# dherrera1911/sqfa

Hardware: AMD Instinct MI355X
Metric: SPD pairwise-distance loss+grad evals/sec (higher is better)
Workload: dtype f32; 1 GPU; c3: C=1000 classes, n_dim=784, n_filters=16, smsqfa (m=16), 499500 unordered pairs per eval, inputs resident in HBM; parallelism=pair-tile shard over 1 GPU(s) + 1 all-reduce of [loss,flags,grad] per eval

## Files before the change

sqfa_amd/csrc/pair_inst.hip:

```cpp
#include <type_traits>

#include "configs.hpp"
#include "pair_kernel.hpp"

#define SQFA_CAT_(a, b, c) a##b##_##c
#define SQFA_CAT(a, b, c) SQFA_CAT_(a, b, c)

#if defined(SQFA_RS) && SQFA_RS != 0
#include "pair_kernel_2d.hpp"
#define SQFA_ROW2D_MATCHES(T, MR, GC, CPL, TJ, WV, RS) \
  || (std::is_same<T, SQFA_T>::value && MR == SQFA_MR && GC == SQFA_G && CPL == SQFA_CPL && TJ == SQFA_TJ && WV == SQFA_WAVES && RS == SQFA_RS)
static_assert(false SQFA_CONFIGS2D_F32(SQFA_ROW2D_MATCHES) SQFA_CONFIGS2D_F64(SQFA_ROW2D_MATCHES),
              "Makefile CONFIGS2D and configs.hpp disagree");
namespace sqfa {
hipError_t SQFA_CAT(launch_pair2d_, SQFA_TAG, SQFA_MR)(const PairParams& p, hipStream_t stream) {
  return launch_pair_tiles_2d<PairCfg2D<SQFA_T, SQFA_MR, SQFA_G, SQFA_CPL, SQFA_TJ, SQFA_WAVES, SQFA_RS>>(p, stream);
}
hipError_t SQFA_CAT(launch_pair2d_bw_, SQFA_TAG, SQFA_MR)(const PairParams& p, hipStream_t stream) {
  return launch_pair_tiles_2d_bw<PairCfg2D<SQFA_T, SQFA_MR, SQFA_G, SQFA_CPL, SQFA_TJ, SQFA_WAVES, SQFA_RS>>(p, stream);
}
hipError_t SQFA_CAT(launch_factor2d_, SQFA_TAG, SQFA_MR)(const PairParams& p, hipStream_t stream) {
  return launch_class_factors<PairCfg2D<SQFA_T, SQFA_MR, SQFA_G, SQFA_CPL, SQFA_TJ, SQFA_WAVES, SQFA_RS>>(p, stream);
}
hipError_t SQFA_CAT(launch_classeig2d_, SQFA_TAG, SQFA_MR)(const void* LT, int n, int m, double* U, double* lam, hipStream_t stream) {
  return launch_class_eig<PairCfg2D<SQFA_T, SQFA_MR, SQFA_G, SQFA_CPL, SQFA_TJ, SQFA_WAVES, SQFA_RS>>(LT, n, m, U, lam, stream);
}
}
#else
#define SQFA_ROW_MATCHES(T, MR, G, CPL, TJ, WV) \
  || (std::is_same<T, SQFA_T>::value && MR == SQFA_MR && G == SQFA_G && CPL == SQFA_CPL && TJ == SQFA_TJ && WV == SQFA_WAVES)
static_assert(false SQFA_CONFIGS_F32(SQFA_ROW_MATCHES) SQFA_CONFIGS_F64(SQFA_ROW_MATCHES) SQFA_CONFIGS_F32_SMALL(SQFA_ROW_MATCHES)
              SQFA_CONFIGS_F64_SMALL(SQFA_ROW_MATCHES),
              "Makefile CONFIGS / CONFIGS_SMALL and configs.hpp disagree");
namespace sqfa {
hipError_t SQFA_CAT(launch_pair_, SQFA_TAG, SQFA_MR)(const PairParams& p, hipStream_t stream) {
  return launch_pair_tiles<PairCfg<SQFA_T, SQFA_MR, SQFA_G, SQFA_CPL, SQFA_TJ, SQFA_WAVES>>(p, stream);
}
hipError_t SQFA_CAT(launch_pair_bw_, SQFA_TAG, SQFA_MR)(const PairParams& p, hipStream_t stream) {
  return launch_pair_tiles_bw<PairCfg<SQFA_T, SQFA_MR, SQFA_G, SQFA_CPL, SQFA_TJ, SQFA_WAVES>>(p, stream);
}
hipError_t SQFA_CAT(launch_factor_, SQFA_TAG, SQFA_MR)(const PairParams& p, hipStream_t stream) {
  return launch_class_factors<PairCfg<SQFA_T, SQFA_MR, SQFA_G, SQFA_CPL, SQFA_TJ, SQFA_WAVES>>(p, stream);
}
hipError_t SQFA_CAT(launch_classeig_, SQFA_TAG, SQFA_MR)(const void* LT, int n, int m, double* U, double* lam, hipStream_t stream) {
  return launch_class_eig<PairCfg<SQFA_T, SQFA_MR, SQFA_G, SQFA_CPL, SQFA_TJ, SQFA_WAVES>>(LT, n, m, U, lam, stream);
}
}
#endif
```

sqfa_amd/csrc/pair_kernel.hpp:

```cpp
#pragma once
#include <hip/hip_runtime.h>
#include <stdint.h>

namespace sqfa {

struct PairParams {
  const void* LT;
  const void* Linv;
  const void* W;
  const void* EW;
  void* slab_grad;
  void* slab_loss;
  int* slab_flag;
  int* row_start;
  void* dist_out;
  void* eig_out;
  unsigned long long* sweep_counter;
  int nA, nB, m;
  int self_mode, sqrt_mode, want_grad;
  int shard_index, shard_count;
  int nbi, nbj;
  int tj;
  int factor_mode;
  const double* mean_linv;
// ... 7 lines not shown
template <typename T> __device__ __forceinline__ T param_scale(const PairParams& p) {
  if constexpr (sizeof(T) == 4) return p.scale_f; else return p.scale;
}
template <typename T> __device__ __forceinline__ T param_eps(const PairParams& p) {
  if constexpr (sizeof(T) == 4) return p.eps_f; else return p.eps;
}
template <typename T> __device__ __forceinline__ T param_uniform_weight(const PairParams& p) {
  if constexpr (sizeof(T) == 4) return p.uniform_weight_f; else return p.uniform_weight;
}

__host__ __device__ inline int tiles_in_row(int bi, int nbj, int TI, int TJ, int self_mode) {
  if (!self_mode) return nbj;
  const int q = bi * TI + TI - 2;
  if (q < 0) return 0;
  const int len = q / TJ + 1;
  return len < nbj ? len : nbj;
}
__host__ __device__ inline int shard_tiles_in_row(int bi, int len, int shard_index, int shard_count, int* first) {
  const int o = ((shard_index - bi) % shard_count + shard_count) % shard_count;
  *first = o;
  return len > o ? (len - 1 - o) / shard_count + 1 : 0;
}

__device__ inline void write_row_start_table(const PairParams& pp, int TI, int* row_start) {
  __shared__ int s_cnt[256];
  int base = 0;
  for (int b0 = 0; b0 < pp.nbi; b0 += 256) {
    const int bi = b0 + (int)threadIdx.x;
    int cnt = 0, first;
    if (bi < pp.nbi)
      cnt = shard_tiles_in_row(bi, tiles_in_row(bi, pp.nbj, TI, pp.tj, pp.self_mode), pp.shard_index, pp.shard_count, &first);
    s_cnt[threadIdx.x] = cnt;
    __syncthreads();
    if (threadIdx.x == 0) {
      int acc = base;
      for (int k = 0; k < 256 && b0 + k < pp.nbi; ++k) {
        row_start[b0 + k] = acc;
        acc += s_cnt[k];
      }
      s_cnt[0] = acc;
    }
    __syncthreads();
    base = s_cnt[0];
    __syncthreads();
  }
  if (threadIdx.x == 0) row_start[pp.nbi] = base;
}

__host__ __device__ constexpr int ilog2(int v);
__host__ __device__ constexpr int pow2ceil(int v) {
  int p = 1;
  while (p < v) p <<= 1;
  return p;
}
__host__ __device__ constexpr int tri_index(int r, int c) { return r * (r + 1) / 2 + c; }

template <typename T> struct Real;
template <> struct Real<float> {
  static constexpr float kEps = 1.1920929e-07f;
// ... 1276 lines not shown
  return hipGetLastError();
}

template <typename Cfg>
hipError_t launch_pair_tiles(const PairParams& p, hipStream_t stream) {
  long n_tiles = 0;
  for (int bi = 0; bi < p.nbi; ++bi) {
    int first;
    n_tiles += shard_tiles_in_row(bi, tiles_in_row(bi, p.nbj, Cfg::TI, p.tj, p.self_mode), p.shard_index,
                                  p.shard_count, &first);
  }
  if (n_tiles == 0) return hipSuccess;
  dim3 grid((unsigned)n_tiles, 1, 1);
  using T = typename Cfg::type;
  if (p.EW != nullptr)
    hipLaunchKernelGGL((pair_tile_kernel<Cfg, true>), grid, dim3(Cfg::THREADS), 0, stream, p, static_cast<const T*>(p.LT),
                       static_cast<const T*>(p.Linv), static_cast<const T*>(p.W), static_cast<const T*>(p.EW));
  else
    hipLaunchKernelGGL((pair_tile_kernel<Cfg, false>), grid, dim3(Cfg::THREADS), 0, stream, p, static_cast<const T*>(p.LT),
                       static_cast<const T*>(p.Linv), static_cast<const T*>(p.W), static_cast<const T*>(p.EW));
  return hipGetLastError();
}

#ifndef SQFA_FACTOR_F64
#define SQFA_FACTOR_F64 1
#endif
template <typename Tio_, int MR_>
struct FactorCfg {
  using io_type = Tio_;
  static constexpr int MR = MR_;
#ifndef SQFA_FACTOR_G
  static constexpr int G = MR_ <= 24 ? 16 : 32;
#else
  static constexpr int G = SQFA_FACTOR_G;
#endif
  static constexpr int CPL = (MR_ + G - 1) / G;
  static constexpr int PPW = 64 / G;
};

template <typename T, int MR, int G, int CPL, int ROWS = MR>
__device__ __forceinline__ int class_jacobi_sweeps(T (&x)[CPL][ROWS], T (&D)[CPL], int max_sweeps) {
  using R = Real<T>;
  constexpr bool LONE = (MR == G * (CPL - 1) + 1);
  const T tol2 = R::kEps * R::kEps * T(MR);
  T nrm[CPL];
  int sweeps = 0;
  bool more = true;
  while (more && sweeps < max_sweeps) {
    {
// ... 38 lines not shown
            x[c2][r] = R::fma_(a2, xp, x[c2][r]);
          }
          D[c1] *= u;
          D[c2] *= u;
          nrm[c1] -= kg2;
          nrm[c2] += kg2;
        }
      }
    }
    constexpr int STATIC_G = sizeof(T) == 4 ? 32 : 16;
    if constexpr (G > 1 && G <= STATIC_G) {
      cross_rounds_static<T, ROWS, G, CPL, 1, LONE ? 1 : 0>(x, nrm, D, tol2, big);
    } else if constexpr (G > STATIC_G) {
#pragma unroll 1
      for (int s = 1; s < G; ++s) cross_round<T, ROWS, CPL, 0, 0, LONE>(x, nrm, D, s, tol2, big);
    }
    if constexpr (z_visits_cfg<G, MR, CPL>()) z_visits<T, ROWS, G, CPL, swizzled_rows_of_8<T, G, MR>(), 0>(x, nrm, D, tol2, big);
    more = __any(big);
    ++sweeps;
  }
  return sweeps;
}

template <typename Cfg>
__global__ __launch_bounds__(64) void class_factor_kernel(typename Cfg::io_type* __restrict__ LT, int nA, int max_sweeps) {
  using Tio = typename Cfg::io_type;
#if SQFA_FACTOR_F64
  using T = double;
#else
  using T = Tio;
#endif
  using R = Real<T>;
  constexpr int MR = Cfg::MR, G = Cfg::G, CPL = Cfg::CPL, PPW = Cfg::PPW;
  const int lane = threadIdx.x & 63;
  const int g = lane % G;
  const int cls = blockIdx.x * PPW + lane / G;
  Tio* lt = LT + (size_t)(cls < nA ? cls : nA - 1) * (MR * MR);
  T x[CPL][MR];
#pragma unroll
  for (int c = 0; c < CPL; ++c) {
    const int col = c * G + g;
    const Tio* src = lt + (size_t)(col < MR ? col : 0) * MR;
    const bool real_col = col < MR;
#pragma unroll
    for (int k = 0; k < MR; ++k) x[c][k] = real_col ? (T)src[k] : T(0);
  }
  T D[CPL];
#pragma unroll
  for (int c = 0; c < CPL; ++c) D[c] = T(1);
  class_jacobi_sweeps<T, MR, G, CPL>(x, D, max_sweeps);
  if (cls < nA) {
#pragma unroll
    for (int c = 0; c < CPL; ++c) {
      const int col = c * G + g;
      if (col < MR) {
        const T dc = R::sqrt_(D[c]);
        Tio* dst = lt + (size_t)col * MR;
#pragma unroll
        for (int r = 0; r < MR; ++r) dst[r] = (Tio)(x[c][r] * dc);
      }
    }
  }
}

template <typename Cfg>
__global__ __launch_bounds__(64) void class_factor_mean_kernel(typename Cfg::io_type* __restrict__ LT, int nA, int max_sweeps,
                                                               const double* __restrict__ mean_linv) {
  using Tio = typename Cfg::io_type;
  using T = double;
  using R = Real<T>;
  constexpr int MR = Cfg::MR, G = Cfg::G, CPL = Cfg::CPL, PPW = Cfg::PPW, ROWS = 2 * MR;
  constexpr T kStack = T(1.0 / (1 << 30)), kUnstack = T(1 << 30);
  __shared__ T s_li[MR * MR];
  const int lane = threadIdx.x & 63;
  for (int k = lane; k < MR * MR; k += 64) s_li[k] = mean_linv[k];
  __syncthreads();
  const int g = lane % G;
  const int cls = blockIdx.x * PPW + lane / G;
  Tio* lt = LT + (size_t)(cls < nA ? cls : nA - 1) * (MR * MR);
  T x[CPL][ROWS];
#pragma unroll
  for (int c = 0; c < CPL; ++c) {
// ... 64 lines not shown
        for (int r = 0; r < MR; ++r) a = R::fma_(x[c][r], x[c][r], a);
        const T l = a * D[c];
        lam[(size_t)cls * m + col] = l;
        const T inv = R::sqrt_(D[c]) / R::sqrt_(l);
#pragma unroll
        for (int r = 0; r < MR; ++r) {
          if (r < m) U[((size_t)cls * m + r) * m + col] = x[c][r] * inv;
        }
      }
    }
  }
}

template <typename Cfg>
hipError_t launch_class_eig(const void* LT, int n, int m, double* U, double* lam, hipStream_t stream) {
  using T = typename Cfg::type;
  using FC = FactorCfg<T, Cfg::MR>;
  const int blocks = (n + FC::PPW - 1) / FC::PPW;
  hipLaunchKernelGGL((class_eig_kernel<FC>), dim3(blocks), dim3(64), 0, stream, static_cast<const T*>(LT), n, m, U, lam);
  return hipGetLastError();
}

template <typename Cfg>
hipError_t launch_class_factors(const PairParams& p, hipStream_t stream) {
  if constexpr (!Cfg::DENSE_FACTOR) {
    return hipSuccess;
  } else {
    using T = typename Cfg::type;
    using FC = FactorCfg<T, Cfg::MR>;
    const long pairs = p.self_mode ? (long)p.nA * (p.nA - 1) / 2 : (long)p.nA * p.nB;
    if (p.factor_mode < 0 || (p.factor_mode == 0 && pairs / p.shard_count < Cfg::FACTOR_MIN_PAIRS)) return hipSuccess;
    const int blocks = (p.nA + FC::PPW - 1) / FC::PPW;
    if constexpr (Cfg::MEAN_METRIC) {
      if (p.mean_linv != nullptr) {
        hipLaunchKernelGGL((class_factor_mean_kernel<FC>), dim3(blocks), dim3(64), 0, stream,
                           static_cast<T*>(const_cast<void*>(p.LT)), p.nA, Cfg::FACTOR_SWEEPS, p.mean_linv);
        return hipGetLastError();
      }
    }
    hipLaunchKernelGGL((class_factor_kernel<FC>), dim3(blocks), dim3(64), 0, stream,
                       static_cast<T*>(const_cast<void*>(p.LT)), p.nA, Cfg::FACTOR_SWEEPS);
    return hipGetLastError();
  }
}

}
```

sqfa_amd/csrc/sqfa_api.hip:

```cpp
#include <hip/hip_runtime.h>
#include <stdio.h>
#include <string.h>

#include <algorithm>
#include <atomic>
#include <mutex>
#include <utility>
#include <vector>

#include "../../include/sqfa_hip.h"
#include "configs.hpp"
#include "pair_kernel.hpp"
#include "pair_kernel_2d.hpp"
#include "pair_kernel_lds.hpp"

namespace sqfa {

#define SQFA_DECL_F32(T, MR, G, CPL, TJ, WV) \
  hipError_t launch_pair_f32_##MR(const PairParams&, hipStream_t);   \
  hipError_t launch_pair_bw_f32_##MR(const PairParams&, hipStream_t); \
  hipError_t launch_factor_f32_##MR(const PairParams&, hipStream_t); \
  hipError_t launch_classeig_f32_##MR(const void*, int, int, double*, double*, hipStream_t);
#define SQFA_DECL_F64(T, MR, G, CPL, TJ, WV) \
  hipError_t launch_pair_f64_##MR(const PairParams&, hipStream_t);   \
  hipError_t launch_pair_bw_f64_##MR(const PairParams&, hipStream_t); \
  hipError_t launch_factor_f64_##MR(const PairParams&, hipStream_t); \
  hipError_t launch_classeig_f64_##MR(const void*, int, int, double*, double*, hipStream_t);
SQFA_CONFIGS_F32(SQFA_DECL_F32)
SQFA_CONFIGS_F64(SQFA_DECL_F64)
#define SQFA_DECL_F32S(T, MR, G, CPL, TJ, WV) \
  hipError_t launch_pair_f32s_##MR(const PairParams&, hipStream_t);  \
  hipError_t launch_pair_bw_f32s_##MR(const PairParams&, hipStream_t); \
  hipError_t launch_factor_f32s_##MR(const PairParams&, hipStream_t);
SQFA_CONFIGS_F32_SMALL(SQFA_DECL_F32S)
#define SQFA_DECL_F64S(T, MR, G, CPL, TJ, WV) \
  hipError_t launch_pair_f64s_##MR(const PairParams&, hipStream_t);  \
  hipError_t launch_pair_bw_f64s_##MR(const PairParams&, hipStream_t); \
  hipError_t launch_factor_f64s_##MR(const PairParams&, hipStream_t);
SQFA_CONFIGS_F64_SMALL(SQFA_DECL_F64S)

#define SQFA_DECL2D_F32(T, MR, GC, CPL, TJ, WV, RS) \
  hipError_t launch_pair2d_f32_##MR(const PairParams&, hipStream_t); \
  hipError_t launch_pair2d_bw_f32_##MR(const PairParams&, hipStream_t); \
  hipError_t launch_factor2d_f32_##MR(const PairParams&, hipStream_t); \
  hipError_t launch_classeig2d_f32_##MR(const void*, int, int, double*, double*, hipStream_t);
#define SQFA_DECL2D_F64(T, MR, GC, CPL, TJ, WV, RS) \
  hipError_t launch_pair2d_f64_##MR(const PairParams&, hipStream_t); \
  hipError_t launch_pair2d_bw_f64_##MR(const PairParams&, hipStream_t); \
  hipError_t launch_factor2d_f64_##MR(const PairParams&, hipStream_t); \
  hipError_t launch_classeig2d_f64_##MR(const void*, int, int, double*, double*, hipStream_t);
SQFA_CONFIGS2D_F32(SQFA_DECL2D_F32)
SQFA_CONFIGS2D_F64(SQFA_DECL2D_F64)

struct Geometry {
  int dtype, MR, TJ, TI, WV;
  hipError_t (*launch)(const PairParams&, hipStream_t);
  hipError_t (*factor)(const PairParams&, hipStream_t);
  hipError_t (*eig)(const void*, int, int, double*, double*, hipStream_t);
  hipError_t (*launch_bw)(const PairParams&, hipStream_t);
  bool mean_metric;
  long factor_min_pairs;
};
template <typename Cfg>
static Geometry make_geometry(decltype(Geometry::launch) launch, decltype(Geometry::factor) factor, decltype(Geometry::eig) eig,
                              decltype(Geometry::launch_bw) launch_bw) {
  return Geometry{sizeof(typename Cfg::type) == 4 ? SQFA_F32 : SQFA_F64, Cfg::MR, Cfg::TJ, Cfg::TI, Cfg::WAVES, launch, factor, eig,
                  launch_bw, Cfg::MEAN_METRIC, Cfg::FACTOR_MIN_PAIRS};
}

static bool find_geometry(int m, int dtype, long pairs, Geometry* out, int geometry_mode = 0) {
  bool found = false;
  Geometry best{};
  auto consider = [&](const Geometry& g) {
    if (g.dtype == dtype && m <= g.MR && (!found || g.MR < best.MR)) {
      best = g;
      found = true;
    }
  };
  auto consider_small = [&](Geometry g, long max_pairs) {
    g.eig = best.eig;
    if (g.dtype == dtype && g.MR == best.MR && (geometry_mode > 0 || pairs < max_pairs)) best = g;
  };
#define SQFA_ROW_F32(T, MR, G, CPL, TJ, WV) \
  consider(make_geometry<PairCfg<T, MR, G, CPL, TJ, WV>>(launch_pair_f32_##MR, launch_factor_f32_##MR, launch_classeig_f32_##MR, launch_pair_bw_f32_##MR));
#define SQFA_ROW_F64(T, MR, G, CPL, TJ, WV) \
  consider(make_geometry<PairCfg<T, MR, G, CPL, TJ, WV>>(launch_pair_f64_##MR, launch_factor_f64_##MR, launch_classeig_f64_##MR, launch_pair_bw_f64_##MR));
#define SQFA_ROW2D_F32(T, MR, GC, CPL, TJ, WV, RS) \
  consider(make_geometry<PairCfg2D<T, MR, GC, CPL, TJ, WV, RS>>(launch_pair2d_f32_##MR, launch_factor2d_f32_##MR, launch_classeig2d_f32_##MR, launch_pair2d_bw_f32_##MR));
#define SQFA_ROW2D_F64(T, MR, GC, CPL, TJ, WV, RS) \
  consider(make_geometry<PairCfg2D<T, MR, GC, CPL, TJ, WV, RS>>(launch_pair2d_f64_##MR, launch_factor2d_f64_##MR, launch_classeig2d_f64_##MR, launch_pair2d_bw_f64_##MR));
#define SQFA_ROW_F32S(T, MR, G, CPL, TJ, WV) \
  consider_small(make_geometry<PairCfg<T, MR, G, CPL, TJ, WV>>(launch_pair_f32s_##MR, launch_factor_f32s_##MR, nullptr, launch_pair_bw_f32s_##MR), small_launch_max_pairs(MR));
#define SQFA_ROW_F64S(T, MR, G, CPL, TJ, WV) \
  consider_small(make_geometry<PairCfg<T, MR, G, CPL, TJ, WV>>(launch_pair_f64s_##MR, launch_factor_f64s_##MR, nullptr, launch_pair_bw_f64s_##MR), small_launch_max_pairs_f64(MR));
  SQFA_CONFIGS_F32(SQFA_ROW_F32)
  SQFA_CONFIGS_F64(SQFA_ROW_F64)
  SQFA_CONFIGS2D_F32(SQFA_ROW2D_F32)
  SQFA_CONFIGS2D_F64(SQFA_ROW2D_F64)
  if (found && geometry_mode >= 0 && pairs >= 0) {
    SQFA_CONFIGS_F32_SMALL(SQFA_ROW_F32S)
    SQFA_CONFIGS_F64_SMALL(SQFA_ROW_F64S)
  }
  if (found) *out = best;
  return found;
}
static long pair_count(int nA, int nB, int shard_count) {
  const long p = nB == 0 ? (long)nA * (nA - 1) / 2 : (long)nA * nB;
  return p / (shard_count > 0 ? shard_count : 1);
}

constexpr int kSpdMaxDim = kRegMaxDim;

static thread_local char g_last_error[256] = "";

struct EventPair { hipEvent_t a, b; };
static std::atomic<bool> g_profile{false};
static std::vector<EventPair> g_events;
// ... 128 lines not shown
  if (pl.lds) {
    if (m > kLdsMaxDim) return false;
    pl.MR = lds_padded_size(m);
    pl.TI = pl.TJ = 16;
    while (pl.TI * pl.TJ > 4 && shard_tiles(nA, pl.nBeff, pl.TI, pl.TJ, pl.self_mode, 0, 1) < kLdsMinTiles) {
      if (pl.TJ >= pl.TI) pl.TJ /= 2;
      else pl.TI /= 2;
    }
    pl.tj = pl.TJ;
  } else {
    if (!find_geometry(m, dtype, pair_count(nA, nB, shard_count), &pl.g, geometry_mode)) return false;
    pl.MR = pl.g.MR;
    pl.TI = pl.g.TI;
    pl.TJ = pl.g.TJ;
    pl.tj = choose_tile_width(nA, pl.nBeff, pl.g, pl.self_mode, shard_count);
  }
  pl.nbi = (nA + pl.TI - 1) / pl.TI;
  pl.nbj = (pl.nBeff + pl.tj - 1) / pl.tj;
  pl.w = pl.lds ? layout_lds(pl) : layout(pl, any_width);
  *out = pl;
  return true;
}

__device__ __forceinline__ double fast_rsqrt(double x) {
  double y = __builtin_amdgcn_rsq(x);
  y = y * (1.5 - 0.5 * x * y * y);
  y = y * (1.5 - 0.5 * x * y * y);
  return y;
}

template <typename T>
__global__ __launch_bounds__(256) void mean_partial_kernel(const T* __restrict__ S, int n, int m, double* __restrict__ out) {
  const int b = blockIdx.x, P = gridDim.x;
  for (int e = threadIdx.x; e < m * m; e += 256) {
    double a0 = 0.0, a1 = 0.0;
    int c = b;
    for (; c + P < n; c += 2 * P) {
      a0 += (double)S[(size_t)c * m * m + e];
      a1 += (double)S[(size_t)(c + P) * m * m + e];
    }
    if (c < n) a0 += (double)S[(size_t)c * m * m + e];
    out[(size_t)b * m * m + e] = a0 + a1;
  }
}

template <typename T, int MAXM>
__global__ __launch_bounds__(256) void cholesky_kernel(const T* __restrict__ S, int m, int MR,
                                                       T* __restrict__ LT, T* __restrict__ Linv,
                                                       int* __restrict__ row_start, PairParams pp, int TI,
                                                       int n_classes = 0, const double* __restrict__ mean_parts = nullptr,
                                                       int n_parts = 0, double* __restrict__ mean_linv = nullptr) {
  if (row_start != nullptr && blockIdx.x == 0) write_row_start_table(pp, TI, row_start);
// ... 512 lines not shown
  p.eps = eps;
  p.uniform_weight = uniform_weight;
  p.scale_f = (float)scale;
  p.eps_f = (float)eps;
  p.uniform_weight_f = (float)uniform_weight;
  return p;
}

static void launch_cholesky(int dtype, int m, hipStream_t stream, const void* S, int n, int MR, void* LT, void* Linv,
                            int* row_start, const PairParams& p, int TI, const double* mean_parts = nullptr, int n_parts = 0,
                            double* mean_linv = nullptr) {
  const int blocks = n + (mean_parts != nullptr ? 1 : 0);
  auto launch = [&](auto zero) {
    using T = decltype(zero);
    auto kernel = m <= 16 ? cholesky_kernel<T, 16> : (m <= 32 ? cholesky_kernel<T, 32> : cholesky_kernel<T, 64>);
    hipLaunchKernelGGL(kernel, dim3(blocks), dim3(256), 0, stream, static_cast<const T*>(S), m, MR, static_cast<T*>(LT),
                       static_cast<T*>(Linv), row_start, p, TI, n, mean_parts, n_parts, mean_linv);
  };
  if (dtype == SQFA_F32) launch(0.0f);
  else launch(0.0);
}

static hipError_t launch_factors(const PairPlan& pl, const PairParams& p, hipStream_t stream, const void* S, int n, void* LT,
                                 void* Linv, int* row_start, const double* mean_parts = nullptr, int n_parts = 0,
                                 double* mean_linv = nullptr) {
  if (pl.lds) return launch_lds_prologue(pl.dtype == SQFA_F64, S, n, pl.m, pl.MR, LT, Linv, row_start, p, pl.TI, stream);
  launch_cholesky(pl.dtype, pl.m, stream, S, n, pl.MR, LT, Linv, row_start, p, pl.TI, mean_parts, n_parts, mean_linv);
  return hipGetLastError();
}

template <typename F>
static hipError_t launch_profiled(hipStream_t stream, F launch) {
  bool prof = g_profile.load();
  if (prof) {
    hipStreamCaptureStatus cap = hipStreamCaptureStatusNone;
    if (hipStreamIsCapturing(stream, &cap) != hipSuccess || cap != hipStreamCaptureStatusNone) prof = false;
  }
  EventPair ev{};
  if (prof) {
    (void)hipEventCreate(&ev.a);
    (void)hipEventCreate(&ev.b);
    (void)hipEventRecord(ev.a, stream);
  }
  const hipError_t e = launch();
  if (prof) {
    (void)hipEventRecord(ev.b, stream);
    std::lock_guard<std::mutex> lock(g_events_mutex);
    g_events.push_back(ev);
  }
// ... 99 lines not shown
  if (rc != SQFA_OK) return rc;
  PairPlan pl;
  if (!make_plan(nA, nB, m, dtype, shard_count, options ? clamp_policy(options->geometry_policy) : 0, &pl))
    return fail(SQFA_ERR_UNSUPPORTED_M, "matrix size not supported", hipSuccess);
  if (workspace_bytes < pl.w.total) return fail(SQFA_ERR_WORKSPACE, "workspace too small", hipSuccess);
  char* ws = static_cast<char*>(workspace);
  PairParams p = make_pair_params(pl, ws, shard_index, scale, eps, sqrt_mode, pair_weights, uniform_weight, gradA_out != nullptr,
                                  dist_out, options);
  p.EW = eig_weights;
  p.eig_out = eig_out;

  const int mean_mode = options ? clamp_policy(options->mean_metric_policy) : 0;
  const bool want_mean = pl.g.mean_metric && mean_mode > 0 && p.factor_mode >= 0 &&
                         (p.factor_mode > 0 || pair_count(nA, nB, shard_count) >= pl.g.factor_min_pairs) && nA >= 2;
  double* mean_parts = reinterpret_cast<double*>(ws + pl.w.off_mean);
  double* mean_linv = mean_parts + (size_t)kMeanParts * pl.MR * pl.MR;
  const int n_parts = nA < kMeanParts ? nA : kMeanParts;
  if (want_mean) {
    if (dtype == SQFA_F32) hipLaunchKernelGGL(mean_partial_kernel<float>, dim3(n_parts), dim3(256), 0, stream, static_cast<const float*>(A), nA, m, mean_parts);
    else hipLaunchKernelGGL(mean_partial_kernel<double>, dim3(n_parts), dim3(256), 0, stream, static_cast<const double*>(A), nA, m, mean_parts);
    p.mean_linv = mean_linv;
  }
  hipError_t e = launch_factors(pl, p, stream, A, nA, ws + pl.w.off_lt, pl.self_mode ? ws + pl.w.off_linv : nullptr, p.row_start,
                                want_mean ? mean_parts : nullptr, n_parts, mean_linv);
  if (!pl.self_mode && e == hipSuccess) e = launch_factors(pl, p, stream, B, nB, nullptr, ws + pl.w.off_linv, nullptr);
  if (e != hipSuccess) return fail(SQFA_ERR_LAUNCH, pl.lds ? "cholesky_lds_kernel" : "cholesky_kernel", e);
  if (pl.g.factor != nullptr) {
    e = pl.g.factor(p, stream);
    if (e != hipSuccess) return fail(SQFA_ERR_LAUNCH, "class_factor_kernel", e);
  }

  e = launch_profiled(stream, [&] { return pl.lds ? launch_pair_lds(dtype == SQFA_F64, p, pl.TI, pl.MR, stream) : pl.g.launch(p, stream); });
  if (e != hipSuccess) return fail(SQFA_ERR_LAUNCH, pl.lds ? "pair_lds_kernel" : "pair_tile_kernel", e);

  e = launch_finalize(pl, p, gradA_out, gradB_out, loss_out, nonfinite_out, stream);
  if (e != hipSuccess) return fail(SQFA_ERR_LAUNCH, "finalize_kernel", e);
  return SQFA_OK;
}

struct BwExtra {
  size_t off_tr, off_h, off_hsum, off_sinv, off_g, off_w, total;
};
static void bw_tiles(int nA, int nB, int m, int dtype, int* nbi, int* TJ) {
  PairPlan regular, small;
  make_plan(nA, nB, m, dtype, 1, -1, &regular);
  make_plan(nA, nB, m, dtype, 1, 1, &small);
  *nbi = std::max(regular.nbi, small.nbi);
  *TJ = std::max(regular.TJ, small.TJ);
}
static BwExtra bw_extra(size_t base, int nA, int nB, int m, int dtype) {
  const int nBeff = nB == 0 ? nA : nB;
  int nbi, TJ;
// ... 11 lines not shown
}

static int bw_impl(const void* A, int nA, const void* B, int nB, int m, int dtype, double eps, int sqrt_mode,
                   const void* pair_weights, double uniform_weight, int shard_index, int shard_count, void* loss_out,
                   void* gradA_out, void* gradB_out, void* dist_out, int* nonfinite_out, void* workspace,
                   size_t workspace_bytes, void* stream_, const sqfa_airm_options* options) {
  hipStream_t stream = static_cast<hipStream_t>(stream_);
  const int rc = validate_pair_call(A, nA, B, nB, m, dtype, shard_index, shard_count, workspace);
  if (rc != SQFA_OK) return rc;
  PairPlan pl;
  if (!make_plan(nA, nB, m, dtype, shard_count, options ? clamp_policy(options->geometry_policy) : 0, &pl))
    return fail(SQFA_ERR_UNSUPPORTED_M, "matrix size not supported", hipSuccess);
  const BwExtra x = bw_extra(pl.w.total, nA, nB, m, dtype);
  if (workspace_bytes < x.total) return fail(SQFA_ERR_WORKSPACE, "workspace too small", hipSuccess);
  char* ws = static_cast<char*>(workspace);
  double* tr = reinterpret_cast<double*>(ws + x.off_tr);
  double* sinv = reinterpret_cast<double*>(ws + x.off_sinv);
  PairParams p = make_pair_params(pl, ws, shard_index, 1.0, eps, sqrt_mode, pair_weights, uniform_weight, gradA_out != nullptr,
                                  dist_out, options);
  p.trA = tr;
  p.trB = pl.self_mode ? tr : tr + nA;
  p.slab_h = ws + x.off_h;

  hipError_t e = launch_factors(pl, p, stream, A, nA, ws + pl.w.off_lt, nullptr, p.row_start);
  if (e != hipSuccess) return fail(SQFA_ERR_LAUNCH, "cholesky_kernel", e);
  auto by_dtype = [&](auto launch) {
    if (dtype == SQFA_F32) launch(0.0f);
    else launch(0.0);
    return hipGetLastError();
  };
  e = by_dtype([&](auto zero) {
    using T = decltype(zero);
    const size_t lds_bytes = ((size_t)m * (m + 1) + m) * sizeof(double);
    if (lds_bytes > 64 * 1024)
      (void)hipFuncSetAttribute(reinterpret_cast<const void*>(bw_prologue_kernel<T>), hipFuncAttributeMaxDynamicSharedMemorySize, (int)lds_bytes);
    auto launch = [&](const void* S, int n, void* R, double* si, double* trace) {
      hipLaunchKernelGGL(bw_prologue_kernel<T>, dim3(n), dim3(256), lds_bytes, stream, static_cast<const T*>(S), m, pl.MR,
                         static_cast<T*>(R), si, trace);
    };
    void* rslot = ws + pl.w.off_linv;
    if (pl.self_mode) launch(A, nA, rslot, sinv, tr);
    else { launch(A, nA, nullptr, nullptr, tr); launch(B, nB, rslot, sinv, tr + nA); }
  });
  if (e != hipSuccess) return fail(SQFA_ERR_LAUNCH, "bw_prologue_kernel", e);
  if (pl.g.factor != nullptr) {
    e = pl.g.factor(p, stream);
    if (e != hipSuccess) return fail(SQFA_ERR_LAUNCH, "class_factor_kernel", e);
  }

  e = launch_profiled(stream, [&] { return pl.lds ? launch_pair_lds_bw(dtype == SQFA_F64, p, pl.TI, pl.MR, stream) : pl.g.launch_bw(p, stream); });
  if (e != hipSuccess) return fail(SQFA_ERR_LAUNCH, "pair_tile_kernel (Bures-Wasserstein)", e);

  PairParams q = p;
  q.want_grad = 0;
  e = launch_finalize(pl, q, nullptr, nullptr, loss_out, nonfinite_out, stream);
  if (e != hipSuccess) return fail(SQFA_ERR_LAUNCH, "finalize_kernel", e);
  if (p.want_grad) {
    double* G = reinterpret_cast<double*>(ws + x.off_g);
    double* W = reinterpret_cast<double*>(ws + x.off_w);
    double* hs = reinterpret_cast<double*>(ws + x.off_hsum);
    void* outB = pl.self_mode ? gradA_out : gradB_out;
    e = by_dtype([&](auto zero) {
      using T = decltype(zero);
      hipLaunchKernelGGL(finalize_bw_kernel<T>, dim3((nA + pl.nBeff) * finalize_bw_bpc(pl.MR * (pl.MR + 1) / 2)), dim3(256), 0, stream,
                         p, pl.TI, pl.tj, pl.MR, static_cast<T*>(gradA_out), G, hs);
      if (outB != nullptr)
        hipLaunchKernelGGL(bw_sandwich_kernel<T>, dim3(pl.nBeff), dim3(256), 0, stream, m, sinv, G, W, hs, static_cast<T*>(outB),
                           pl.self_mode);
    });
    if (e != hipSuccess) return fail(SQFA_ERR_LAUNCH, "finalize_bw_kernel", e);
  }
// ... 119 lines not shown
```

Baseline: 1431 evals/s.

## Fuse Cholesky, inverse and Jacobi class-factor pass into one prologue kernel

Replaces the separate Cholesky launch and the follow-up class_factor_kernel with a single class_prologue_kernel. Each wave factors one class in LDS in double precision, writes Linv and the row-start table, and optionally runs the Jacobi sweeps on the in-LDS factor before writing LT. This removes one kernel launch and the global round trip of LT between the factor and sweep stages. In exchange it adds a new LDS-based Cholesky with its own occupancy limits, and the mean-metric path stays separate.

```diff
diff --git a/sqfa_amd/csrc/pair_inst.hip b/sqfa_amd/csrc/pair_inst.hip
--- a/sqfa_amd/csrc/pair_inst.hip
+++ b/sqfa_amd/csrc/pair_inst.hip
@@ -20,7 +20,12 @@
   return launch_pair_tiles_2d_bw<PairCfg2D<SQFA_T, SQFA_MR, SQFA_G, SQFA_CPL, SQFA_TJ, SQFA_WAVES, SQFA_RS>>(p, stream);
 }
 hipError_t SQFA_CAT(launch_factor2d_, SQFA_TAG, SQFA_MR)(const PairParams& p, hipStream_t stream) {
-  return launch_class_factors<PairCfg2D<SQFA_T, SQFA_MR, SQFA_G, SQFA_CPL, SQFA_TJ, SQFA_WAVES, SQFA_RS>>(p, stream);
+  return launch_class_factors_mean<PairCfg2D<SQFA_T, SQFA_MR, SQFA_G, SQFA_CPL, SQFA_TJ, SQFA_WAVES, SQFA_RS>>(p, stream);
+}
+hipError_t SQFA_CAT(launch_prologue2d_, SQFA_TAG, SQFA_MR)(const PairParams& p, const void* S, int n, void* LT, void* Linv,
+                                                            int* row_start, bool factor_pass, hipStream_t stream) {
+  return launch_class_prologue<PairCfg2D<SQFA_T, SQFA_MR, SQFA_G, SQFA_CPL, SQFA_TJ, SQFA_WAVES, SQFA_RS>>(p, S, n, LT, Linv, row_start,
+                                                                                                            factor_pass, stream);
 }
 hipError_t SQFA_CAT(launch_classeig2d_, SQFA_TAG, SQFA_MR)(const void* LT, int n, int m, double* U, double* lam, hipStream_t stream) {
   return launch_class_eig<PairCfg2D<SQFA_T, SQFA_MR, SQFA_G, SQFA_CPL, SQFA_TJ, SQFA_WAVES, SQFA_RS>>(LT, n, m, U, lam, stream);
@@ -40,7 +45,12 @@
   return launch_pair_tiles_bw<PairCfg<SQFA_T, SQFA_MR, SQFA_G, SQFA_CPL, SQFA_TJ, SQFA_WAVES>>(p, stream);
 }
 hipError_t SQFA_CAT(launch_factor_, SQFA_TAG, SQFA_MR)(const PairParams& p, hipStream_t stream) {
-  return launch_class_factors<PairCfg<SQFA_T, SQFA_MR, SQFA_G, SQFA_CPL, SQFA_TJ, SQFA_WAVES>>(p, stream);
+  return launch_class_factors_mean<PairCfg<SQFA_T, SQFA_MR, SQFA_G, SQFA_CPL, SQFA_TJ, SQFA_WAVES>>(p, stream);
+}
+hipError_t SQFA_CAT(launch_prologue_, SQFA_TAG, SQFA_MR)(const PairParams& p, const void* S, int n, void* LT, void* Linv,
+                                                          int* row_start, bool factor_pass, hipStream_t stream) {
+  return launch_class_prologue<PairCfg<SQFA_T, SQFA_MR, SQFA_G, SQFA_CPL, SQFA_TJ, SQFA_WAVES>>(p, S, n, LT, Linv, row_start, factor_pass,
+                                                                                                 stream);
 }
 hipError_t SQFA_CAT(launch_classeig_, SQFA_TAG, SQFA_MR)(const void* LT, int n, int m, double* U, double* lam, hipStream_t stream) {
   return launch_class_eig<PairCfg<SQFA_T, SQFA_MR, SQFA_G, SQFA_CPL, SQFA_TJ, SQFA_WAVES>>(LT, n, m, U, lam, stream);
diff --git a/sqfa_amd/csrc/pair_kernel.hpp b/sqfa_amd/csrc/pair_kernel.hpp
--- a/sqfa_amd/csrc/pair_kernel.hpp
+++ b/sqfa_amd/csrc/pair_kernel.hpp
@@ -53,10 +53,10 @@
   return len > o ? (len - 1 - o) / shard_count + 1 : 0;
 }
 
-__device__ inline void write_row_start_table(const PairParams& pp, int TI, int* row_start) {
+__device__ inline void write_row_start_table(const PairParams& pp, int TI, int* row_start, int nthreads = 256) {
   __shared__ int s_cnt[256];
   int base = 0;
-  for (int b0 = 0; b0 < pp.nbi; b0 += 256) {
+  for (int b0 = 0; b0 < pp.nbi; b0 += nthreads) {
     const int bi = b0 + (int)threadIdx.x;
     int cnt = 0, first;
     if (bi < pp.nbi)
@@ -65,7 +65,7 @@
     __syncthreads();
     if (threadIdx.x == 0) {
       int acc = base;
-      for (int k = 0; k < 256 && b0 + k < pp.nbi; ++k) {
+      for (int k = 0; k < nthreads && b0 + k < pp.nbi; ++k) {
         row_start[b0 + k] = acc;
         acc += s_cnt[k];
       }
@@ -1388,9 +1388,6 @@
   return hipGetLastError();
 }
 
-#ifndef SQFA_FACTOR_F64
-#define SQFA_FACTOR_F64 1
-#endif
 template <typename Tio_, int MR_>
 struct FactorCfg {
   using io_type = Tio_;
@@ -1475,42 +1472,138 @@
   return sweeps;
 }
 
-template <typename Cfg>
-__global__ __launch_bounds__(64) void class_factor_kernel(typename Cfg::io_type* __restrict__ LT, int nA, int max_sweeps) {
+__device__ __forceinline__ double fast_rsqrt(double x) {
+  double y = __builtin_amdgcn_rsq(x);
+  y = y * (1.5 - 0.5 * x * y * y);
+  y = y * (1.5 - 0.5 * x * y * y);
+  return y;
+}
+
+#ifndef SQFA_FACTOR_F64
+#define SQFA_FACTOR_F64 1
+#endif
+template <typename Tio_, int MR_>
+struct PrologueCfg : FactorCfg<Tio_, MR_> {
+  static constexpr int PITCH = MR_ + 1;
+  static constexpr int WAVE_DOUBLES = MR_ * PITCH + MR_;
+  static constexpr int WAVES = WAVE_DOUBLES * 8 * 4 <= 40960 ? 4 : (WAVE_DOUBLES * 8 * 2 <= 40960 ? 2 : 1);
+  static constexpr int P2 = pow2ceil(MR_);
+};
+
+template <typename Cfg, bool SWEEPS>
+__global__ __launch_bounds__(64 * Cfg::WAVES) void class_prologue_kernel(const typename Cfg::io_type* __restrict__ S, int n, int m,
+                                                                          typename Cfg::io_type* __restrict__ LT,
+                                                                          typename Cfg::io_type* __restrict__ Linv, int max_sweeps,
+                                                                          int* __restrict__ row_start, PairParams pp, int TI) {
   using Tio = typename Cfg::io_type;
+  constexpr int MR = Cfg::MR, G = Cfg::G, CPL = Cfg::CPL, PITCH = Cfg::PITCH, P2 = Cfg::P2, LP2 = ilog2(Cfg::P2);
+  if (row_start != nullptr && blockIdx.x == 0) write_row_start_table(pp, TI, row_start, 64 * Cfg::WAVES);
+  __shared__ double s_cls[Cfg::WAVES * Cfg::WAVE_DOUBLES];
+  const int lane = threadIdx.x & 63;
+  const int wave = __builtin_amdgcn_readfirstlane((int)(threadIdx.x >> 6));
+  const int c = blockIdx.x * Cfg::WAVES + wave;
+  if (c >= n) return;
+  double* ab = s_cls + wave * Cfg::WAVE_DOUBLES;
+  double* rd = ab + MR * PITCH;
+  auto a_at = [&](int r, int k) -> double& { return ab[r * PITCH + k]; };
+  auto b_at = [&](int r, int k) -> double& { return ab[k * PITCH + r + 1]; };
+  auto wave_sync = [] {
+    __builtin_amdgcn_fence(__ATOMIC_ACQ_REL, "wavefront");
+    __builtin_amdgcn_wave_barrier();
+  };
+  {
+    const Tio* s = S + (size_t)c * m * m;
+    for (int idx = lane; idx < m * m; idx += 64) {
+      const int r = idx / m, k = idx % m;
+      if (k <= r) a_at(r, k) = (double)s[idx];
+    }
+  }
+  wave_sync();
+  for (int k = 0; k < m; ++k) {
+    const double akk = a_at(k, k);
+    double rk = __builtin_amdgcn_rcp(akk);
+    rk = rk * (2.0 - akk * rk);
+    rk = rk * (2.0 - akk * rk);
+    if (!(akk > 0.0)) rk = __builtin_nan("");
+    const int nt = m - k - 1;
+    for (int e = lane; e < nt * P2; e += 64) {
+      const int dr = e >> LP2, dc = e & (P2 - 1);
+      const int r = k + 1 + dr, c2 = k + 1 + dc;
+      if (dc <= dr) a_at(r, c2) -= a_at(r, k) * a_at(c2, k) * rk;
+    }
+    wave_sync();
+  }
+  for (int k = lane; k < m; k += 64) rd[k] = fast_rsqrt(a_at(k, k));
+  wave_sync();
+  for (int e = lane; e < m * P2; e += 64) {
+    const int r = e >> LP2, k = e & (P2 - 1);
+    if (k <= r) a_at(r, k) *= rd[k];
+  }
+  wave_sync();
+  if (Linv != nullptr) {
+    const int part = lane & 3;
+    for (int r = 0; r < m; ++r) {
+      for (int col = lane >> 2; col <= r; col += 16) {
+        double acc = 0.0;
+        if (col < r) {
+          for (int k = col + part; k < r; k += 4) acc += a_at(r, k) * b_at(k, col);
+        }
+        acc += __shfl_xor(acc, 1, 64);
+        acc += __shfl_xor(acc, 2, 64);
+        if (part == 0) b_at(r, col) = ((col == r ? 1.0 : 0.0) - acc) * rd[r];
+      }
+      wave_sync();
+    }
+    for (int idx = lane; idx < MR * MR; idx += 64) {
+      const int r = idx / MR, k = idx % MR;
+      if (k > r && Cfg::MR >= 32) continue;
+      const double v = (r < m && k < m) ? (k <= r ? b_at(r, k) : 0.0) : (r == k ? 1.0 : 0.0);
+      if (MR >= 32) Linv[(size_t)c * (MR * (MR + 1) / 2) + tri_index(r, k)] = (Tio)v;
+      else Linv[(size_t)c * (MR * MR) + idx] = (Tio)v;
+    }
+  }
+  if (LT == nullptr) return;
+  Tio* lt = LT + (size_t)c * (MR * MR);
+  auto factor_at = [&](int col, int k) -> Tio {
+    const double v = (col < m && k < m) ? (k >= col ? a_at(k, col) : 0.0) : (col == k ? 1.0 : 0.0);
+    return (Tio)v;
+  };
+  if constexpr (!SWEEPS) {
+    for (int idx = lane; idx < MR * MR; idx += 64) lt[idx] = factor_at(idx / MR, idx % MR);
+  } else {
 #if SQFA_FACTOR_F64
-  using T = double;
+    using T = double;
 #else
-  using T = Tio;
-#endif
-  using R = Real<T>;
-  constexpr int MR = Cfg::MR, G = Cfg::G, CPL = Cfg::CPL, PPW = Cfg::PPW;
-  const int lane = threadIdx.x & 63;
-  const int g = lane % G;
-  const int cls = blockIdx.x * PPW + lane / G;
-  Tio* lt = LT + (size_t)(cls < nA ? cls : nA - 1) * (MR * MR);
-  T x[CPL][MR];
-#pragma unroll
-  for (int c = 0; c < CPL; ++c) {
-    const int col = c * G + g;
-    const Tio* src = lt + (size_t)(col < MR ? col : 0) * MR;
-    const bool real_col = col < MR;
-#pragma unroll
-    for (int k = 0; k < MR; ++k) x[c][k] = real_col ? (T)src[k] : T(0);
-  }
-  T D[CPL];
-#pragma unroll
-  for (int c = 0; c < CPL; ++c) D[c] = T(1);
-  class_jacobi_sweeps<T, MR, G, CPL>(x, D, max_sweeps);
-  if (cls < nA) {
-#pragma unroll
-    for (int c = 0; c < CPL; ++c) {
-      const int col = c * G + g;
-      if (col < MR) {
-        const T dc = R::sqrt_(D[c]);
-        Tio* dst = lt + (size_t)col * MR;
-#pragma unroll
-        for (int r = 0; r < MR; ++r) dst[r] = (Tio)(x[c][r] * dc);
+    using T = Tio;
+#endif
+    using R = Real<T>;
+    const int g = lane % G;
+    T x[CPL][MR];
+#pragma unroll
+    for (int cs = 0; cs < CPL; ++cs) {
+      const int col = cs * G + g;
+      const bool real_col = col < MR;
+      const int colr = real_col ? col : 0;
+#pragma unroll
+      for (int k = 0; k < MR; ++k) {
+        const double v = (colr < m && k < m) ? (k >= colr ? ab[k * PITCH + (k >= colr ? colr : 0)] : 0.0) : (colr == k ? 1.0 : 0.0);
+        x[cs][k] = real_col ? (T)(Tio)v : T(0);
+      }
+    }
+    T D[CPL];
+#pragma unroll
+    for (int cs = 0; cs < CPL; ++cs) D[cs] = T(1);
+    class_jacobi_sweeps<T, MR, G, CPL>(x, D, max_sweeps);
+    if (lane < G) {
+#pragma unroll
+      for (int cs = 0; cs < CPL; ++cs) {
+        const int col = cs * G + g;
+        if (col < MR) {
+          const T dc = R::sqrt_(D[cs]);
+          Tio* dst = lt + (size_t)col * MR;
+#pragma unroll
+          for (int r = 0; r < MR; ++r) dst[r] = (Tio)(x[cs][r] * dc);
+        }
       }
     }
   }
@@ -1621,26 +1714,44 @@
 }
 
 template <typename Cfg>
-hipError_t launch_class_factors(const PairParams& p, hipStream_t stream) {
-  if constexpr (!Cfg::DENSE_FACTOR) {
+bool class_factor_pass_wanted(const PairParams& p) {
+  if (!Cfg::DENSE_FACTOR || p.factor_mode < 0) return false;
+  const long pairs = p.self_mode ? (long)p.nA * (p.nA - 1) / 2 : (long)p.nA * p.nB;
+  return p.factor_mode > 0 || pairs / p.shard_count >= Cfg::FACTOR_MIN_PAIRS;
+}
+
+template <typename Cfg>
+hipError_t launch_class_factors_mean(const PairParams& p, hipStream_t stream) {
+  if constexpr (!Cfg::MEAN_METRIC) {
     return hipSuccess;
   } else {
     using T = typename Cfg::type;
     using FC = FactorCfg<T, Cfg::MR>;
-    const long pairs = p.self_mode ? (long)p.nA * (p.nA - 1) / 2 : (long)p.nA * p.nB;
-    if (p.factor_mode < 0 || (p.factor_mode == 0 && pairs / p.shard_count < Cfg::FACTOR_MIN_PAIRS)) return hipSuccess;
+    if (p.mean_linv == nullptr || !class_factor_pass_wanted<Cfg>(p)) return hipSuccess;
     const int blocks = (p.nA + FC::PPW - 1) / FC::PPW;
-    if constexpr (Cfg::MEAN_METRIC) {
-      if (p.mean_linv != nullptr) {
-        hipLaunchKernelGGL((class_factor_mean_kernel<FC>), dim3(blocks), dim3(64), 0, stream,
-                           static_cast<T*>(const_cast<void*>(p.LT)), p.nA, Cfg::FACTOR_SWEEPS, p.mean_linv);
-        return hipGetLastError();
-      }
-    }
-    hipLaunchKernelGGL((class_factor_kernel<FC>), dim3(blocks), dim3(64), 0, stream,
-                       static_cast<T*>(const_cast<void*>(p.LT)), p.nA, Cfg::FACTOR_SWEEPS);
+    hipLaunchKernelGGL((class_factor_mean_kernel<FC>), dim3(blocks), dim3(64), 0, stream,
+                       static_cast<T*>(const_cast<void*>(p.LT)), p.nA, Cfg::FACTOR_SWEEPS, p.mean_linv);
     return hipGetLastError();
   }
 }
 
-}
+template <typename Cfg>
+hipError_t launch_class_prologue(const PairParams& p, const void* S, int n, void* LT, void* Linv, int* row_start,
+                                 bool factor_pass, hipStream_t stream) {
+  using T = typename Cfg::type;
+  using PC = PrologueCfg<T, Cfg::MR>;
+  const dim3 grid((n + PC::WAVES - 1) / PC::WAVES), block(64 * PC::WAVES);
+  bool sweeps = false;
+  if constexpr (Cfg::DENSE_FACTOR) {
+    sweeps = factor_pass && LT != nullptr && class_factor_pass_wanted<Cfg>(p);
+    if (sweeps)
+      hipLaunchKernelGGL((class_prologue_kernel<PC, true>), grid, block, 0, stream, static_cast<const T*>(S), n, p.m,
+                         static_cast<T*>(LT), static_cast<T*>(Linv), Cfg::FACTOR_SWEEPS, row_start, p, Cfg::TI);
+  }
+  if (!sweeps)
+    hipLaunchKernelGGL((class_prologue_kernel<PC, false>), grid, block, 0, stream, static_cast<const T*>(S), n, p.m,
+                       static_cast<T*>(LT), static_cast<T*>(Linv), 0, row_start, p, Cfg::TI);
+  return hipGetLastError();
+}
+
+}
diff --git a/sqfa_amd/csrc/sqfa_api.hip b/sqfa_amd/csrc/sqfa_api.hip
--- a/sqfa_amd/csrc/sqfa_api.hip
+++ b/sqfa_amd/csrc/sqfa_api.hip
@@ -20,34 +20,40 @@
   hipError_t launch_pair_f32_##MR(const PairParams&, hipStream_t);   \
   hipError_t launch_pair_bw_f32_##MR(const PairParams&, hipStream_t); \
   hipError_t launch_factor_f32_##MR(const PairParams&, hipStream_t); \
+  hipError_t launch_prologue_f32_##MR(const PairParams&, const void*, int, void*, void*, int*, bool, hipStream_t); \
   hipError_t launch_classeig_f32_##MR(const void*, int, int, double*, double*, hipStream_t);
 #define SQFA_DECL_F64(T, MR, G, CPL, TJ, WV) \
   hipError_t launch_pair_f64_##MR(const PairParams&, hipStream_t);   \
   hipError_t launch_pair_bw_f64_##MR(const PairParams&, hipStream_t); \
   hipError_t launch_factor_f64_##MR(const PairParams&, hipStream_t); \
+  hipError_t launch_prologue_f64_##MR(const PairParams&, const void*, int, void*, void*, int*, bool, hipStream_t); \
   hipError_t launch_classeig_f64_##MR(const void*, int, int, double*, double*, hipStream_t);
 SQFA_CONFIGS_F32(SQFA_DECL_F32)
 SQFA_CONFIGS_F64(SQFA_DECL_F64)
 #define SQFA_DECL_F32S(T, MR, G, CPL, TJ, WV) \
   hipError_t launch_pair_f32s_##MR(const PairParams&, hipStream_t);  \
   hipError_t launch_pair_bw_f32s_##MR(const PairParams&, hipStream_t); \
-  hipError_t launch_factor_f32s_##MR(const PairParams&, hipStream_t);
+  hipError_t launch_factor_f32s_##MR(const PairParams&, hipStream_t); \
+  hipError_t launch_prologue_f32s_##MR(const PairParams&, const void*, int, void*, void*, int*, bool, hipStream_t);
 SQFA_CONFIGS_F32_SMALL(SQFA_DECL_F32S)
 #define SQFA_DECL_F64S(T, MR, G, CPL, TJ, WV) \
   hipError_t launch_pair_f64s_##MR(const PairParams&, hipStream_t);  \
   hipError_t launch_pair_bw_f64s_##MR(const PairParams&, hipStream_t); \
-  hipError_t launch_factor_f64s_##MR(const PairParams&, hipStream_t);
+  hipError_t launch_factor_f64s_##MR(const PairParams&, hipStream_t); \
+  hipError_t launch_prologue_f64s_##MR(const PairParams&, const void*, int, void*, void*, int*, bool, hipStream_t);
 SQFA_CONFIGS_F64_SMALL(SQFA_DECL_F64S)
 
 #define SQFA_DECL2D_F32(T, MR, GC, CPL, TJ, WV, RS) \
   hipError_t launch_pair2d_f32_##MR(const PairParams&, hipStream_t); \
   hipError_t launch_pair2d_bw_f32_##MR(const PairParams&, hipStream_t); \
   hipError_t launch_factor2d_f32_##MR(const PairParams&, hipStream_t); \
+  hipError_t launch_prologue2d_f32_##MR(const PairParams&, const void*, int, void*, void*, int*, bool, hipStream_t); \
   hipError_t launch_classeig2d_f32_##MR(const void*, int, int, double*, double*, hipStream_t);
 #define SQFA_DECL2D_F64(T, MR, GC, CPL, TJ, WV, RS) \
   hipError_t launch_pair2d_f64_##MR(const PairParams&, hipStream_t); \
   hipError_t launch_pair2d_bw_f64_##MR(const PairParams&, hipStream_t); \
   hipError_t launch_factor2d_f64_##MR(const PairParams&, hipStream_t); \
+  hipError_t launch_prologue2d_f64_##MR(const PairParams&, const void*, int, void*, void*, int*, bool, hipStream_t); \
   hipError_t launch_classeig2d_f64_##MR(const void*, int, int, double*, double*, hipStream_t);
 SQFA_CONFIGS2D_F32(SQFA_DECL2D_F32)
 SQFA_CONFIGS2D_F64(SQFA_DECL2D_F64)
@@ -58,14 +64,15 @@
   hipError_t (*factor)(const PairParams&, hipStream_t);
   hipError_t (*eig)(const void*, int, int, double*, double*, hipStream_t);
   hipError_t (*launch_bw)(const PairParams&, hipStream_t);
+  hipError_t (*prologue)(const PairParams&, const void*, int, void*, void*, int*, bool, hipStream_t);
   bool mean_metric;
   long factor_min_pairs;
 };
 template <typename Cfg>
 static Geometry make_geometry(decltype(Geometry::launch) launch, decltype(Geometry::factor) factor, decltype(Geometry::eig) eig,
-                              decltype(Geometry::launch_bw) launch_bw) {
+                              decltype(Geometry::launch_bw) launch_bw, decltype(Geometry::prologue) prologue) {
   return Geometry{sizeof(typename Cfg::type) == 4 ? SQFA_F32 : SQFA_F64, Cfg::MR, Cfg::TJ, Cfg::TI, Cfg::WAVES, launch, factor, eig,
-                  launch_bw, Cfg::MEAN_METRIC, Cfg::FACTOR_MIN_PAIRS};
+                  launch_bw, prologue, Cfg::MEAN_METRIC, Cfg::FACTOR_MIN_PAIRS};
 }
 
 static bool find_geometry(int m, int dtype, long pairs, Geometry* out, int geometry_mode = 0) {
@@ -82,17 +89,17 @@
     if (g.dtype == dtype && g.MR == best.MR && (geometry_mode > 0 || pairs < max_pairs)) best = g;
   };
 #define SQFA_ROW_F32(T, MR, G, CPL, TJ, WV) \
-  consider(make_geometry<PairCfg<T, MR, G, CPL, TJ, WV>>(launch_pair_f32_##MR, launch_factor_f32_##MR, launch_classeig_f32_##MR, launch_pair_bw_f32_##MR));
+  consider(make_geometry<PairCfg<T, MR, G, CPL, TJ, WV>>(launch_pair_f32_##MR, launch_factor_f32_##MR, launch_classeig_f32_##MR, launch_pair_bw_f32_##MR, launch_prologue_f32_##MR));
 #define SQFA_ROW_F64(T, MR, G, CPL, TJ, WV) \
-  consider(make_geometry<PairCfg<T, MR, G, CPL, TJ, WV>>(launch_pair_f64_##MR, launch_factor_f64_##MR, launch_classeig_f64_##MR, launch_pair_bw_f64_##MR));
+  consider(make_geometry<PairCfg<T, MR, G, CPL, TJ, WV>>(launch_pair_f64_##MR, launch_factor_f64_##MR, launch_classeig_f64_##MR, launch_pair_bw_f64_##MR, launch_prologue_f64_##MR));
 #define SQFA_ROW2D_F32(T, MR, GC, CPL, TJ, WV, RS) \
-  consider(make_geometry<PairCfg2D<T, MR, GC, CPL, TJ, WV, RS>>(launch_pair2d_f32_##MR, launch_factor2d_f32_##MR, launch_classeig2d_f32_##MR, launch_pair2d_bw_f32_##MR));
+  consider(make_geometry<PairCfg2D<T, MR, GC, CPL, TJ, WV, RS>>(launch_pair2d_f32_##MR, launch_factor2d_f32_##MR, launch_classeig2d_f32_##MR, launch_pair2d_bw_f32_##MR, launch_prologue2d_f32_##MR));
 #define SQFA_ROW2D_F64(T, MR, GC, CPL, TJ, WV, RS) \
-  consider(make_geometry<PairCfg2D<T, MR, GC, CPL, TJ, WV, RS>>(launch_pair2d_f64_##MR, launch_factor2d_f64_##MR, launch_classeig2d_f64_##MR, launch_pair2d_bw_f64_##MR));
+  consider(make_geometry<PairCfg2D<T, MR, GC, CPL, TJ, WV, RS>>(launch_pair2d_f64_##MR, launch_factor2d_f64_##MR, launch_classeig2d_f64_##MR, launch_pair2d_bw_f64_##MR, launch_prologue2d_f64_##MR));
 #define SQFA_ROW_F32S(T, MR, G, CPL, TJ, WV) \
-  consider_small(make_geometry<PairCfg<T, MR, G, CPL, TJ, WV>>(launch_pair_f32s_##MR, launch_factor_f32s_##MR, nullptr, launch_pair_bw_f32s_##MR), small_launch_max_pairs(MR));
+  consider_small(make_geometry<PairCfg<T, MR, G, CPL, TJ, WV>>(launch_pair_f32s_##MR, launch_factor_f32s_##MR, nullptr, launch_pair_bw_f32s_##MR, launch_prologue_f32s_##MR), small_launch_max_pairs(MR));
 #define SQFA_ROW_F64S(T, MR, G, CPL, TJ, WV) \
-  consider_small(make_geometry<PairCfg<T, MR, G, CPL, TJ, WV>>(launch_pair_f64s_##MR, launch_factor_f64s_##MR, nullptr, launch_pair_bw_f64s_##MR), small_launch_max_pairs_f64(MR));
+  consider_small(make_geometry<PairCfg<T, MR, G, CPL, TJ, WV>>(launch_pair_f64s_##MR, launch_factor_f64s_##MR, nullptr, launch_pair_bw_f64s_##MR, launch_prologue_f64s_##MR), small_launch_max_pairs_f64(MR));
   SQFA_CONFIGS_F32(SQFA_ROW_F32)
   SQFA_CONFIGS_F64(SQFA_ROW_F64)
   SQFA_CONFIGS2D_F32(SQFA_ROW2D_F32)
@@ -267,12 +274,6 @@
   return true;
 }
 
-__device__ __forceinline__ double fast_rsqrt(double x) {
-  double y = __builtin_amdgcn_rsq(x);
-  y = y * (1.5 - 0.5 * x * y * y);
-  y = y * (1.5 - 0.5 * x * y * y);
-  return y;
-}
 
 template <typename T>
 __global__ __launch_bounds__(256) void mean_partial_kernel(const T* __restrict__ S, int n, int m, double* __restrict__ out) {
@@ -831,9 +832,10 @@
 }
 
 static hipError_t launch_factors(const PairPlan& pl, const PairParams& p, hipStream_t stream, const void* S, int n, void* LT,
-                                 void* Linv, int* row_start, const double* mean_parts = nullptr, int n_parts = 0,
+                                 void* Linv, int* row_start, bool factor_pass, const double* mean_parts = nullptr, int n_parts = 0,
                                  double* mean_linv = nullptr) {
   if (pl.lds) return launch_lds_prologue(pl.dtype == SQFA_F64, S, n, pl.m, pl.MR, LT, Linv, row_start, p, pl.TI, stream);
+  if (mean_parts == nullptr) return pl.g.prologue(p, S, n, LT, Linv, row_start, factor_pass, stream);
   launch_cholesky(pl.dtype, pl.m, stream, S, n, pl.MR, LT, Linv, row_start, p, pl.TI, mean_parts, n_parts, mean_linv);
   return hipGetLastError();
 }
@@ -979,12 +981,12 @@
     p.mean_linv = mean_linv;
   }
   hipError_t e = launch_factors(pl, p, stream, A, nA, ws + pl.w.off_lt, pl.self_mode ? ws + pl.w.off_linv : nullptr, p.row_start,
-                                want_mean ? mean_parts : nullptr, n_parts, mean_linv);
-  if (!pl.self_mode && e == hipSuccess) e = launch_factors(pl, p, stream, B, nB, nullptr, ws + pl.w.off_linv, nullptr);
-  if (e != hipSuccess) return fail(SQFA_ERR_LAUNCH, pl.lds ? "cholesky_lds_kernel" : "cholesky_kernel", e);
-  if (pl.g.factor != nullptr) {
+                                true, want_mean ? mean_parts : nullptr, n_parts, mean_linv);
+  if (!pl.self_mode && e == hipSuccess) e = launch_factors(pl, p, stream, B, nB, nullptr, ws + pl.w.off_linv, nullptr, false);
+  if (e != hipSuccess) return fail(SQFA_ERR_LAUNCH, pl.lds ? "cholesky_lds_kernel" : (want_mean ? "cholesky_kernel" : "class_prologue_kernel"), e);
+  if (want_mean) {
     e = pl.g.factor(p, stream);
-    if (e != hipSuccess) return fail(SQFA_ERR_LAUNCH, "class_factor_kernel", e);
+    if (e != hipSuccess) return fail(SQFA_ERR_LAUNCH, "class_factor_mean_kernel", e);
   }
 
   e = launch_profiled(stream, [&] { return pl.lds ? launch_pair_lds(dtype == SQFA_F64, p, pl.TI, pl.MR, stream) : pl.g.launch(p, stream); });
@@ -1042,8 +1044,8 @@
   p.trB = pl.self_mode ? tr : tr + nA;
   p.slab_h = ws + x.off_h;
 
-  hipError_t e = launch_factors(pl, p, stream, A, nA, ws + pl.w.off_lt, nullptr, p.row_start);
-  if (e != hipSuccess) return fail(SQFA_ERR_LAUNCH, "cholesky_kernel", e);
+  hipError_t e = launch_factors(pl, p, stream, A, nA, ws + pl.w.off_lt, nullptr, p.row_start, true);
+  if (e != hipSuccess) return fail(SQFA_ERR_LAUNCH, pl.lds ? "cholesky_lds_kernel" : "class_prologue_kernel", e);
   auto by_dtype = [&](auto launch) {
     if (dtype == SQFA_F32) launch(0.0f);
     else launch(0.0);
@@ -1063,10 +1065,6 @@
     else { launch(A, nA, nullptr, nullptr, tr); launch(B, nB, rslot, sinv, tr + nA); }
   });
   if (e != hipSuccess) return fail(SQFA_ERR_LAUNCH, "bw_prologue_kernel", e);
-  if (pl.g.factor != nullptr) {
-    e = pl.g.factor(p, stream);
-    if (e != hipSuccess) return fail(SQFA_ERR_LAUNCH, "class_factor_kernel", e);
-  }
 
   e = launch_profiled(stream, [&] { return pl.lds ? launch_pair_lds_bw(dtype == SQFA_F64, p, pl.TI, pl.MR, stream) : pl.g.launch_bw(p, stream); });
   if (e != hipSuccess) return fail(SQFA_ERR_LAUNCH, "pair_tile_kernel (Bures-Wasserstein)", e);
```

Result: no change. 1426 evals/s (-0.3%).
